# BaratiLab/GAMD

Measured on AMD Instinct MI355X. Metric: atom-steps/sec (force eval + integrate), 10k-atom LJ box, higher is better.
Workload: dtype f32; 1 GPU; C2: 10 000-atom LJ box, rho*=0.5, L=92.29 A, cutoff 3.0 sigma=10.2 A, fp32, 4 conv layers x 128, random-init weights (seed 0), 1 box per GPU; n_atoms=10000, boxes=1, launch=single process

## Files before the change

### gamd_amd/csrc/conv_edge.hip

```cpp
#include "gamd_common.h"
#include "gamd_internal.h"

#include <cstdlib>

namespace {

constexpr int conv_lds_floats(bool l0) { return 2 * GAMD_WFRAG_FLOATS + 3 * 128; }

template <bool F2, typename Post, typename Mid>
__device__ __forceinline__ void gemm128_post(const f32x4* W, int lane, const f32x16 (&X)[4], f32x16 (&acc)[4], Post post, Mid mid) {
#pragma unroll
    for (int tp = 0; tp < 4; ++tp) {
        if (tp == 1) mid();
#pragma unroll
        for (int t = 0; t < 4; ++t) {
#pragma unroll
            for (int q = 0; q < 4; ++q) {
                const f32x4 w = W[((tp * 4 + t) * 4 + q) * 64 + lane];
#pragma unroll
                for (int j = 0; j < 4; ++j) {
                    const float x = X[t][q * 4 + j];
                    acc[tp] = F2 ? mfma32(x, w[j], acc[tp]) : mfma32(w[j], x, acc[tp]);
                }
                if (tp > 0) post(tp - 1, t * 4 + q);
// ... 8 lines not shown
__device__ __forceinline__ void phase_barrier() {
    asm volatile("s_waitcnt vmcnt(%0) lgkmcnt(0)" ::"n"(N) : "memory");
    __builtin_amdgcn_s_barrier();
}

__device__ __forceinline__ void load_e_tile(const float* __restrict__ e_frag, int tile, int lane, f32x16 (&X)[4]) {
    const f32x4* ef = (const f32x4*)e_frag + (size_t)tile * 16 * 64;
#pragma unroll
    for (int t = 0; t < 4; ++t)
#pragma unroll
        for (int q = 0; q < 4; ++q) {
            const f32x4 v = gamd_load_stream(&ef[(t * 4 + q) * 64 + lane]);
#pragma unroll
            for (int j = 0; j < 4; ++j) X[t][q * 4 + j] = v[j];
        }
}

template <bool TIME, bool L0>
__global__ void __launch_bounds__(512, 2) k_conv_edge(ConvEdgeArgs a) {
    if (a.devflags[DEVFLAG_FROZEN]) return;
    extern __shared__ __attribute__((aligned(16))) float lds[];
    float* buf0 = lds + (L0 ? 3 * 128 : 0);
    float* buf1 = buf0 + GAMD_WFRAG_FLOATS;
    float* vb1 = L0 ? lds : buf1 + GAMD_WFRAG_FLOATS;
    float* vb3 = vb1 + 128;
    float* vb4 = vb3 + 128;
    float* vSD0 = vb4;

    const int tid = threadIdx.x, lane = tid & 63, slot = lane & 31, half = lane >> 5;
    const int wave = __builtin_amdgcn_readfirstlane(tid >> 6);
    const unsigned lane16 = (unsigned)lane * 16u;
    int E = a.counters[CNT_E];
    if ((long long)E > a.e_cap) E = (int)a.e_cap;
    const int n_tiles = (E + GAMD_TILE - 1) / GAMD_TILE;
    const int n_units = (n_tiles + 3) / 4;
    int first, end, step;
    gamd_xcd_range(n_units, blockIdx.x, gridDim.x, first, end, step);
    if (first >= end) return;
    const int n_iter = ((end - first + step - 1) / step + 1) / 2;
    const int wsub = wave & 3, whalf = wave >> 2;
    const bool early = whalf == 0;
    auto tile_of = [&](int it) {
        const int u = first + (2 * it + whalf) * step;
        return (it < n_iter && u < end) ? u * 4 + wsub : n_tiles;
    };
    auto stage = [&](const float* gw, float* buf) { gamd_stage_weight_raw_contig<8>(gw, buf, wave, lane16); };

    long long tacc[16];
#pragma unroll
    for (int i = 0; i < 16; ++i) tacc[i] = 0;
    long long tprev = 0;
#define TMARK(i) do { if (TIME) { const long long tn__ = (long long)__builtin_readcyclecounter(); tacc[i] += tn__ - tprev; tprev = tn__; } } while (0)

    if (tid < 128) {
        vb1[tid] = a.b1[tid]; vb3[tid] = a.b3[tid];
        if (L0) vSD0[tid] = a.S[tid] + a.D[tid];
        else vb4[tid] = a.b4[tid];
    }
    stage(a.w1p, buf0);

    f32x16 RA[4], RB[4], RC[4];
    auto init_b4 = [&]() {
#pragma unroll
        for (int tp = 0; tp < 4; ++tp) {
            const float b = vb4[32 * tp + slot];
#pragma unroll
            for (int r = 0; r < 16; ++r) RC[tp][r] = b;
        }
    };

    int tile = tile_of(0);
    bool active = tile < n_tiles;
    int src = 0, dst = 0;
    {
// ... 101 lines not shown
        asm volatile("" ::"v"(mask), "v"(p0), "v"(src_n));
        TMARK(5);
        if (active) {
            const unsigned bl = (unsigned)__ballot(src != a.zero_row) >> (4 * half);
            const unsigned real = (bl & 0xFu) | ((bl >> 4) & 0xF0u) | ((bl >> 8) & 0xF00u) | ((bl >> 12) & 0xF000u);
#pragma unroll
            for (int tp = 0; tp < 4; ++tp) {
                const float b = vb3[32 * tp + slot];
#pragma unroll
                for (int r = 0; r < 16; ++r) RC[tp][r] = ((real >> r) & 1u) ? b : GAMD_L0_PAD;
            }
            TMARK(7);
            const unsigned keep_bits = ~(mask << 1);
            gemm128_post<true>((const f32x4*)bx, lane, RA, RC, [&](int tp, int r) {
                RC[tp][r] = gamd_l0_acc(RC[tp][r], (r > 0 && ((keep_bits >> r) & 1u)) ? RC[tp][r - 1] : 0.f);
            }, [&]() { FENCE(); if (it + 1 < n_iter) stage(a.w1p, by); FENCE(); });
            pend_ends = mask;
            if (nvalid > 0 && !((mask >> (nvalid - 1)) & 1u)) pend_ends |= 1u << (nvalid - 1);
            pend_p = p0;
            TMARK(10);
        } else {
            if (it + 1 < n_iter) stage(a.w1p, by);
        }
        if (!early) phase_barrier<0>();
        TMARK(11);
        if (active_n) load_e_tile(a.e_frag, tile_n, lane, RA);
        TMARK(12);
        if (early) early_barrier(active_n);
        TMARK(13);
        tile = tile_n; active = active_n; src = src_n;
    }
    } else {
    for (int it = 0; it < n_iter; ++it) {
        const int x0 = tile * GAMD_TILE + 16 * half;
        int nvalid = E - x0;
        nvalid = !active ? 0 : (nvalid >= 16 ? 16 : (nvalid <= 0 ? 0 : nvalid));
        const int tile_n = tile_of(it + 1);
// ... 51 lines not shown
            gemm128_post<false>((const f32x4*)buf0, lane, RC, RB,
                                [&](int tp, int g) { RB[tp][g] = gamd_silu_hw(RB[tp][g]); },
                                [&]() { FENCE(); stage(a.w4p, buf1); FENCE(); });
            TMARK(8);
        } else {
            stage(a.w4p, buf1);
        }
        phase_barrier<0>();
        asm volatile("" ::"v"(mask), "v"(p0), "v"(src_n), "v"(dst_n));
        TMARK(9);
        if (active) {
            init_b4();
            const unsigned keep_bits = ~(mask << 1);
            gemm128_post<true>((const f32x4*)buf1, lane, RB, RC, [&](int tp, int r) {
                RC[tp][r] = gamd_msg_acc(RA[r >> 2][(r & 3) * 4 + tp], RC[tp][r], (r > 0 && ((keep_bits >> r) & 1u)) ? RC[tp][r - 1] : 0.f);
            }, [&]() { FENCE(); if (it + 1 < n_iter) stage(a.w1p, buf0); FENCE(); });
            pend_ends = mask;
            if (nvalid > 0 && !((mask >> (nvalid - 1)) & 1u)) pend_ends |= 1u << (nvalid - 1);
            pend_p = p0;
            TMARK(10);
        } else {
            if (it + 1 < n_iter) stage(a.w1p, buf0);
        }
        if (!early) phase_barrier<0>();
        TMARK(11);
        if (active_n) load_e_tile(a.e_frag, tile_n, lane, RA);
        TMARK(12);
        if (early) early_barrier(active_n);
        TMARK(13);
        tile = tile_n; active = active_n; src = src_n; dst = dst_n;
    }
    }
#undef FENCE
    piece_stores();
    if (TIME && a.tdbg && lane == 0) {
#pragma unroll
        for (int i = 0; i < 16; ++i) a.tdbg[((size_t)blockIdx.x * 8 + wave) * 16 + i] = tacc[i];
    }
#undef TMARK
}

template <bool TIME, bool L0>
int launch(const ConvEdgeArgs& a, int n_blocks, hipStream_t st) {
    const size_t lds = sizeof(float) * conv_lds_floats(L0);
    static PerDeviceOnce once;
    if (int e = gamd_allow_dynamic_lds(once, (int)lds, k_conv_edge<TIME, L0>)) return e;
    hipLaunchKernelGGL((k_conv_edge<TIME, L0>), dim3(n_blocks), dim3(512), lds, st, a);
    GAMD_CHECK_LAUNCH();
    return 0;
// ... 20 lines not shown
```

### gamd_amd/csrc/gamd_api.hip

```cpp
#include "gamd_host.h"

#include <algorithm>
#include <cmath>
#include <cstddef>
#include <cstdlib>
#include <cstring>
#include <deque>

static_assert(sizeof(gamd_config) == 96 && offsetof(gamd_config, n_boxes) == 88 && offsetof(gamd_config, edge_capacity) == 40,
              "gamd_config layout is part of the C ABI (gamd_amd/_lib.py mirrors it)");

namespace {

bool small_path(const gamd_handle* h) { return h->use_small; }

int fill_com(gamd_handle* h, int enabled, MdCom* c) {
    c->enabled = enabled ? 1 : 0;
    c->blocks = std::max(1, std::min(16, (h->n_per_box + 1023) / 1024));
    c->partial = nullptr;
    if (!c->enabled) return 0;
    if (h->com_partial.ensure(sizeof(double) * 4 * (size_t)c->blocks * (size_t)h->n_boxes, true)) return fail(-12, "allocation failed");
    c->partial = h->com_partial.as<double>();
    return 0;
}
// ... 424 lines not shown

    for (int l = 0; l < h->L; ++l) {
        ConvEdgeArgs ca{};
        ca.counters = h->cur_counters;
        ca.devflags = h->devflags.as<int>();
        ca.col = h->col.as<int>(); ca.erow = h->erow.as<int>();
        ca.chunk_piece = h->chunk_piece.as<int>(); ca.chunk_mask = h->chunk_mask.as<unsigned>();
        ca.e_frag = (h->update_edge && l > 0) ? h->e_frag2.as<float>() : h->e_frag.as<float>();
        ca.emb_out = (h->update_edge && l + 1 < h->L) ? h->e_emb.as<float>() : nullptr;
        ca.hn = h->hn.as<float>(); ca.S = h->S.as<float>(); ca.D = h->D.as<float>();
        if (l0 && l == 0) { ca.hn = h->l0_hn.as<float>(); ca.S = h->l0_S.as<float>(); ca.D = h->l0_D.as<float>(); }
        const LayerDev& ld = h->layers[l];
        ca.w1p = ld.w1p; ca.w2p = ld.w2p; ca.w3p = ld.w3p; ca.w4p = ld.w4p; ca.w16p = ld.w16p;
        ca.b1 = ld.b1; ca.b3 = ld.b3; ca.b4 = ld.b4;
        const bool hoist = l == 0 && h->l0_hoist;
        if (hoist) { ca.w3p = ld.w3p_l0; ca.b3 = ld.b3_l0; }
        ca.partial = h->partial.as<float>();
        ca.piece_cap = h->piece_cap;
        ca.sticky = h->sticky_dev;
        ca.e_cap = h->e_cap;
        ca.zero_row = h->n;
#ifdef GAMD_CHECKED
        { static const bool inject = getenv("GAMD_CHK_INJECT") != nullptr; if (inject) ca.zero_row = 0; }
#endif
        ca.tdbg = h->tdbg.as<long long>();
        if ((r = tev_begin(l))) return r;
        r = h->DT > 1 ? launch_conv_edge_wide_d(ca, h->EHT, h->HT, h->DT, h->n_cu, st)
            : h->wide_conv ? (h->cfg.edge_dtype == GAMD_EDGE_F16X3 ? launch_conv_edge_f16x3_wide(ca, h->EHT, h->HT, h->n_cu, st)
                            : h->cfg.edge_dtype == GAMD_EDGE_BF16 ? launch_conv_edge_bf16_wide(ca, h->EHT, h->HT, h->n_cu, st)
                            : (half_quantum && ca.w16p && !ca.emb_out) ? launch_conv_edge_wide16(ca, h->EHT, h->HT, h->n_cu, st)
                            : small_tiles > 0 ? launch_conv_edge_small_wide(ca, h->EHT, h->HT, small_tiles, st)
// ... 176 lines not shown
    if (!cfg || !out) return fail(-22, "null argument");
    if (cfg->n_atoms <= 0) return fail(-22, "n_atoms must be positive");
    if (cfg->n_boxes < 0 || cfg->n_boxes > (1 << 20)) return fail(-22, "n_boxes out of range");
    const int n_boxes = cfg->n_boxes > 1 ? cfg->n_boxes : 1;
    if ((long long)cfg->n_atoms * n_boxes >= (1 << 23) - 1)
        return fail(-22, "n_atoms x n_boxes = %lld: at most %d atoms per handle", (long long)cfg->n_atoms * n_boxes, (1 << 23) - 2);
    if (cfg->n_layers <= 0 || cfg->n_layers > 16) return fail(-22, "n_layers out of range");
    if (!(cfg->cutoff > 0.f)) return fail(-22, "cutoff must be positive");
    if (cfg->edge_dtype != GAMD_EDGE_F32 && cfg->edge_dtype != GAMD_EDGE_BF16 && cfg->edge_dtype != GAMD_EDGE_F16X3)
        return fail(-22, "unknown edge_dtype");
    if (!(cfg->neighbor_skin >= 0.f)) return fail(-22, "neighbor_skin must be >= 0");
    if (cfg->self_loop_mode != GAMD_SELF_LOOP_DGL07_NOOP && cfg->self_loop_mode != GAMD_SELF_LOOP_APPEND_ZERO_FEATURE)
        return fail(-22, "unknown self_loop_mode %d", cfg->self_loop_mode);
    if (cfg->self_loop_mode != GAMD_SELF_LOOP_DGL07_NOOP && cfg->edge_dtype != GAMD_EDGE_F32)
        return fail(-22, "self_loop_mode 1 is built for the fp32 edge dtype only");
    if (cfg->kernel_select & ~(GAMD_KSEL_FORCE_GENERIC_WIDTH | GAMD_KSEL_FORCE_HALF_QUANTUM | GAMD_KSEL_NO_LAYER0_HOIST))
        return fail(-22, "unknown kernel_select bits 0x%x", cfg->kernel_select);
    int ndev = 0;
    if (hipGetDeviceCount(&ndev) != hipSuccess || ndev <= 0)
        return fail(-19, "no HIP device available: libgamd_hip has no CPU fallback");
    if (cfg->device < 0 || cfg->device >= ndev) return fail(-22, "device %d out of range (%d visible)", cfg->device, ndev);
    DeviceGuard guard(cfg->device);
    hipDeviceProp_t prop;
    HIP_TRY(hipGetDeviceProperties(&prop, cfg->device));
    const int H_true = cfg->encoding_size ? cfg->encoding_size : 128, Eh_true = cfg->edge_embedding_dim ? cfg->edge_embedding_dim : 128;
    const int D_true = cfg->hidden_dim ? cfg->hidden_dim : 128;
    if (H_true < 1 || H_true > 256 || Eh_true < 1 || Eh_true > 256)
        return fail(-22, "encoding_size and edge_embedding_dim must be in [1, 256] (got %d, %d)", H_true, Eh_true);
    if (D_true < 1 || D_true > 256) return fail(-22, "hidden_dim must be in [1, 256] (got %d)", D_true);
    const int Dp = D_true <= 128 ? 128 : 256;
    if (Dp > 128 && cfg->edge_dtype != GAMD_EDGE_F32)
// ... 145 lines not shown
    h->finalized = false;
    return 0;
}

int32_t gamd_finalize_weights(gamd_handle* h) {
    if (!h) return fail(-22, "null handle");
    DeviceGuard guard(h->dev);
    InitStream init(h->init_stream);
    const int F = h->n_feat, L = h->L;
    const int64_t H = h->H, Eh = h->Eh, HT = h->HT, EHT = h->EHT;
    const int64_t Ht = h->H_true, Et = h->Eh_true, Dt = h->D_true;
    const int64_t Dp = h->Dp, DT = h->DT;
    const bool expand = !h->cfg.no_expand_edge;
    BlobBuilder bb;
    struct Off { size_t w1p, w2p, w3p, w4p, w16p = 0, b1, b3, b4, elng = 0, elnb = 0, lng, lnb, wsp, wdp, wpdp, bS, bP, wpep, wphip, bphi;
                 size_t w3p_l0 = 0, b3_l0 = 0, m0 = 0, c0 = 0; };
    std::vector<Off> lo(L);
    std::deque<HostTensor> padded;
    auto get = [&](const std::string& nm, std::initializer_list<int64_t> shp, std::initializer_list<int64_t> pad) -> const HostTensor* {
        const HostTensor* t = find_w(h, nm, shp);
        if (!t) return nullptr;
        const std::vector<int64_t> ps(pad);
        if (t->shape == ps) return t;
        HostTensor o;
        o.shape = ps;
        const int64_t r = ps.size() == 2 ? t->shape[0] : 1, c = ps.size() == 2 ? t->shape[1] : t->shape[0];
        const int64_t cp = ps.size() == 2 ? ps[1] : ps[0], rp = ps.size() == 2 ? ps[0] : 1;
        o.data.assign((size_t)(rp * cp), 0.f);
        for (int64_t i = 0; i < r; ++i) std::copy(t->data.begin() + i * c, t->data.begin() + (i + 1) * c, o.data.begin() + i * cp);
        padded.push_back(std::move(o));
        return &padded.back();
// ... 55 lines not shown
    h->norm_bn = norm_bn ? 1 : 0;
    h->l0_hoist = h->cfg.kind == GAMD_KIND_LJ && h->cfg.edge_dtype == GAMD_EDGE_F32 && !h->wide_conv && DT == 1 && !update_edge &&
                  !(h->cfg.kernel_select & GAMD_KSEL_NO_LAYER0_HOIST);
    const HostTensor* emb0 = h->l0_hoist ? get("node_emb", {1, Ht}, {1, H}) : nullptr;
    if (h->l0_hoist && !emb0) return -2;
    auto permute_f2 = [](const HostTensor& w, const HostTensor& b, HostTensor& wo, HostTensor& bo) {
        wo = w;
        bo = b;
        for (int q = 0; q < 4; ++q)
            for (int s = 0; s < 32; ++s) {
                std::copy(w.data.begin() + (size_t)(4 * s + q) * 128, w.data.begin() + (size_t)(4 * s + q + 1) * 128,
                          wo.data.begin() + (size_t)(32 * q + s) * 128);
                bo.data[32 * q + s] = b.data[4 * s + q];
            }
    };
    for (int l = 0; l < L; ++l) {
        const std::string p = "graph_conv.conv." + std::to_string(l);
        const HostTensor *ea0w = get(p + ".edge_affine.mlp_layer.0.weight", {128, Et}, {128, Eh}), *ea0b = get(p + ".edge_affine.mlp_layer.0.bias", {128}, {128});
        const HostTensor *ea2w = get(p + ".edge_affine.mlp_layer.2.weight", {Dt, 128}, {Dp, 128}), *ea2b = get(p + ".edge_affine.mlp_layer.2.bias", {Dt}, {Dp});
        const HostTensor *sw = get(p + ".src_affine.weight", {Dt, Ht}, {Dp, H}), *sb = get(p + ".src_affine.bias", {Dt}, {Dp});
        const HostTensor *dw = get(p + ".dst_affine.weight", {Dt, Ht}, {Dp, H}), *db = get(p + ".dst_affine.bias", {Dt}, {Dp});
        const HostTensor *t1w = get(p + ".theta_edge.mlp_layer.1.weight", {Dt, Dt}, {Dp, Dp}), *t1b = get(p + ".theta_edge.mlp_layer.1.bias", {Dt}, {Dp});
        const HostTensor *t3w = get(p + ".theta_edge.mlp_layer.3.weight", {Ht, Dt}, {H, Dp}), *t3b = get(p + ".theta_edge.mlp_layer.3.bias", {Ht}, {H});
        const HostTensor *pdw = get(p + ".phi_dst.weight", {Dt, Ht}, {Dp, H}), *pdb = get(p + ".phi_dst.bias", {Dt}, {Dp});
        const HostTensor *pew = get(p + ".phi_edge.weight", {Dt, Ht}, {Dp, H}), *peb = get(p + ".phi_edge.bias", {Dt}, {Dp});
        const HostTensor *phw = get(p + ".phi.mlp_layer.1.weight", {Ht, Dt}, {H, Dp}), *phb = get(p + ".phi.mlp_layer.1.bias", {Ht}, {H});
        const HostTensor *ng = get("graph_conv.norm_layers." + std::to_string(l) + ".weight", {Ht}, {H});
        const HostTensor *nb = get("graph_conv.norm_layers." + std::to_string(l) + ".bias", {Ht}, {H});
        if (!ea0w || !ea0b || !ea2w || !ea2b || !sw || !sb || !dw || !db || !t1w || !t1b || !t3w || !t3b || !pdw ||
            !pdb || !pew || !peb || !phw || !phb || !ng || !nb)
// ... 50 lines not shown
                std::fill(row.begin(), row.end(), 0.0);
                double cr = 0.0;
                for (int64_t i = 0; i < H; ++i) {
                    const double a = (double)pew->data[(size_t)(r * H + i)] * hn0[i];
                    if (a == 0.0) continue;
                    for (int64_t k = 0; k < Dp; ++k) row[k] += a * t3w->data[(size_t)(i * Dp + k)];
                    cr += a * t3b->data[i];
                }
                for (int64_t k = 0; k < Dp; ++k) m0.data[(size_t)(r * Dp + k)] = (float)row[k];
                c0.data[r] = (float)cr;
            }
            HostTensor w3f, b3f;
            permute_f2(*t1w, *t1b, w3f, b3f);
            o.w3p_l0 = put_blocks(&w3f, 1, 1);
            o.b3_l0 = put_vec(&b3f);
            o.m0 = put_node(&m0, 1, 1);
            o.c0 = put_vec(&c0);
        }
        HostTensor b4_perm;
        HostTensor w4_perm;
        auto permute_w4 = [&]() {
            permute_f2(*t3w, *t3b, w4_perm, b4_perm);
            t3b = &b4_perm;
        };
        if (bf16_edges) {
            permute_w4();
            o.w1p = put_edge_bf16(ea0w); o.w2p = put_edge_bf16(ea2w); o.w3p = put_edge_bf16(t1w); o.w4p = put_edge_bf16(&w4_perm);
        } else if (f16x3_edges) {
            o.w1p = put_edge_f16x3(ea0w); o.w2p = put_edge_f16x3(ea2w); o.w3p = put_edge_f16x3(t1w); o.w4p = put_edge_f16x3(t3w);
        } else if (bf16_wide) {
// ... 19 lines not shown
            o.w2p = put_blocks(ea2w, (int)DT, 1);
            o.w3p = put_blocks(t1w, (int)DT, (int)DT);
            if (DT > 1) {
                o.w4p = put_blocks(t3w, (int)HT, (int)DT);
            } else if (h->wide_conv) {
                o.w4p = put_blocks(t3w, (int)HT, 1);
                o.w16p = bb.add((size_t)(EHT + 2 + HT) * GAMD_WFRAG_FLOATS);
                size_t at = o.w16p;
                for (int kb = 0; kb < (int)EHT; ++kb, at += GAMD_WFRAG_FLOATS) pack16x(ea0w->data.data() + 128 * kb, bb.host.data() + at, 128 * (int)EHT, true);
                pack16x(ea2w->data.data(), bb.host.data() + at, 128, true); at += GAMD_WFRAG_FLOATS;
                pack16x(t1w->data.data(), bb.host.data() + at, 128, true); at += GAMD_WFRAG_FLOATS;
                for (int ob = 0; ob < (int)HT; ++ob, at += GAMD_WFRAG_FLOATS) pack16x(t3w->data.data() + (size_t)128 * ob * 128, bb.host.data() + at, 128, false);
            } else {
                permute_w4();
                o.w4p = put_blocks(&w4_perm, 1, 1);
            }
        }
        o.b1 = put_vec(ea0b); o.b3 = put_vec(t1b); o.b4 = put_vec(t3b);
        o.lng = put_vec(ng); o.lnb = put_vec(nb);
        if (update_edge) {
            const HostTensor *eg = get(p + ".edge_layer_norm.weight", {Et}, {Eh}), *eb = get(p + ".edge_layer_norm.bias", {Et}, {Eh});
            if (!eg || !eb) return -2;
            o.elng = put_vec(eg); o.elnb = put_vec(eb);
        }
        o.wsp = put_node(sw, (int)DT, (int)HT); o.wdp = put_node(dw, (int)DT, (int)HT); o.wpdp = put_node(pdw, (int)DT, (int)HT);
        o.bS = bb.add((size_t)Dp);
        for (int i = 0; i < (int)Dp; ++i) bb.host[o.bS + i] = (sb->data[i] + db->data[i]) + ea2b->data[i];
        o.bP = bb.add((size_t)Dp);
        for (int i = 0; i < (int)Dp; ++i) bb.host[o.bP + i] = pdb->data[i] + peb->data[i];
        o.wpep = put_node(pew, (int)DT, (int)HT); o.wphip = put_node(phw, (int)HT, (int)DT); o.bphi = put_vec(phb);
// ... 48 lines not shown
    h->length_mean = lm->data[0];
    h->length_std = ls->data[0];
    h->rbf = RbfGrid{};
    if (expand) {
        const double c0 = cen->data[0], delta = ((double)cen->data[39] - c0) / 39.0;
        bool uniform = delta > 0.0;
        for (int k = 0; k < 40 && uniform; ++k)
            uniform = std::fabs((double)cen->data[k] - (c0 + k * delta)) <= 2.5e-7 * std::max(1.0, std::fabs(c0 + k * delta));
        if (uniform) {
            const double gexp = -(1.0 / 0.025) * 1.4426950408889634, s = 2.0 * delta;
            h->rbf = RbfGrid{1, (float)c0, (float)delta, (float)(-2.0 * gexp * s), (float)(gexp * s * s),
                             (float)std::exp2(2.0 * gexp * s * s)};
        }
    }

    if (h->wblob.ensure(sizeof(float) * bb.host.size(), false)) return fail(-12, "weight blob allocation failed");
    HIP_TRY(init_upload(h->wblob.p, bb.host.data(), sizeof(float) * bb.host.size()));
    const float* B = h->wblob.as<float>();
    h->layers.assign(L, LayerDev{});
    for (int l = 0; l < L; ++l) {
        const Off& o = lo[l];
        LayerDev& d = h->layers[l];
        d.w1p = B + o.w1p; d.w2p = B + o.w2p; d.w3p = B + o.w3p; d.w4p = B + o.w4p;
        d.w16p = (h->wide_conv && h->cfg.edge_dtype == GAMD_EDGE_F32 && DT == 1) ? B + o.w16p : nullptr;
        d.b1 = B + o.b1; d.b3 = B + o.b3; d.b4 = B + o.b4;
        d.node.ln_g = B + o.lng; d.node.ln_b = B + o.lnb;
        if (update_edge) { d.e_ln_g = B + o.elng; d.e_ln_b = B + o.elnb; }
        d.node.wsp = B + o.wsp; d.node.wdp = B + o.wdp; d.node.wpdp = B + o.wpdp;
        d.node.bS = B + o.bS; d.node.bP = B + o.bP;
        d.node.wpep = B + o.wpep; d.node.wphip = B + o.wphip; d.node.bphi = B + o.bphi;
        d.node.c0 = nullptr;
        if (l == 0 && h->l0_hoist) {
            d.w3p_l0 = B + o.w3p_l0; d.b3_l0 = B + o.b3_l0;
            d.node.wpep = B + o.m0; d.node.c0 = B + o.c0;
        }
    }
    h->enc_w1p = B + o_e1; h->enc_w2p = B + o_e2; h->enc_w3p = B + o_e3;
    h->enc_b1 = B + o_eb1; h->enc_b2 = B + o_eb2; h->enc_b3 = B + o_eb3;
    h->enc_lng = B + o_elg; h->enc_lnb = B + o_elb; h->centers = B + o_cen;
    h->dec_w1p = B + o_d1; h->dec_b1 = B + o_db1; h->dec_w2 = B + o_d2; h->dec_b2 = B + o_db2;
    h->node_emb = h->cfg.kind == GAMD_KIND_LJ ? B + o_emb : nullptr;
    h->nenc_w = h->cfg.kind == GAMD_KIND_LJ ? nullptr : B + o_nw;
    h->nenc_b = h->cfg.kind == GAMD_KIND_LJ ? nullptr : B + o_nb;
    h->finalized = true;
    return 0;
}

int32_t gamd_set_scaler(gamd_handle* h, double mean, double var) {
// ... 441 lines not shown
```

### gamd_amd/csrc/gamd_host.h

```cpp
#pragma once
#include "../../include/gamd_hip.h"
#include "gamd_common.h"
#include "gamd_internal.h"

#include <cstdarg>
#include <cstdio>
#include <map>
#include <string>
#include <vector>

#pragma GCC visibility push(hidden)

inline thread_local char g_err[512] = "";

inline int fail(int code, const char* fmt, ...) {
    va_list ap;
    va_start(ap, fmt);
    vsnprintf(g_err, sizeof(g_err), fmt, ap);
    va_end(ap);
    return code;
}

#define HIP_TRY(expr)                                                                              \
    do {                                                                                           \
// ... 30 lines not shown
        bytes = want;
        if (zero) {
            e = hipMemsetAsync(p, 0, want, tl_init_stream);
            if (e == hipSuccess) e = hipStreamSynchronize(tl_init_stream);
            if (e != hipSuccess) return (int)e;
        }
        return 0;
    }
    void release() { if (p) (void)hipFree(p); p = nullptr; bytes = 0; }
    template <typename T> T* as() const { return reinterpret_cast<T*>(p); }
};

struct LayerDev {
    const float *w1p, *w2p, *w3p, *w4p, *b1, *b3, *b4;
    const float *w16p = nullptr;
    const float *e_ln_g = nullptr, *e_ln_b = nullptr;
    const float *w3p_l0 = nullptr, *b3_l0 = nullptr;
    NodeLayerW node;
};

struct DeviceGuard {
    int prev = -1;
    bool changed = false;
    explicit DeviceGuard(int dev) {
        if (hipGetDevice(&prev) == hipSuccess && prev != dev) changed = hipSetDevice(dev) == hipSuccess;
    }
    ~DeviceGuard() { if (changed) (void)hipSetDevice(prev); }
    DeviceGuard(const DeviceGuard&) = delete;
    DeviceGuard& operator=(const DeviceGuard&) = delete;
};
// ... 118 lines not shown
```

### gamd_amd/csrc/wide16.hip

```cpp
#include "gamd_common.h"
#include "gamd_internal.h"

namespace {

__device__ __forceinline__ f32x4 mfma16x(float a, float b, f32x4 c) { return __builtin_amdgcn_mfma_f32_16x16x4f32(a, b, c, 0, 0, 0); }

__device__ __forceinline__ void wide16_barrier() {
    asm volatile("s_waitcnt vmcnt(0) lgkmcnt(0)" ::: "memory");
    __builtin_amdgcn_s_barrier();
    asm volatile("" ::: "memory");
}

template <bool F2, int D = 3>
__device__ __forceinline__ void gemm16x(const f32x4* W, int lane, const f32x4 (&X)[8], f32x4 (&acc)[8]) {
    __builtin_amdgcn_sched_barrier(0);
    f32x4 w0[D], w1[D];
#pragma unroll
    for (int s = 0; s < D; ++s) {
        w0[s] = W[((2 * (s >> 3)) * 8 + (s & 7)) * 64 + lane];
        w1[s] = W[((2 * (s >> 3) + 1) * 8 + (s & 7)) * 64 + lane];
    }
#pragma unroll
    for (int s = 0; s < 32; ++s) {
        const int o2 = s >> 3, m4 = s & 7;
        const f32x4 a0 = w0[s % D], a1 = w1[s % D];
#pragma unroll
        for (int c = 0; c < 4; ++c) {
            const float x = X[m4][c];
            acc[2 * o2] = F2 ? mfma16x(x, a0[c], acc[2 * o2]) : mfma16x(a0[c], x, acc[2 * o2]);
            acc[2 * o2 + 1] = F2 ? mfma16x(x, a1[c], acc[2 * o2 + 1]) : mfma16x(a1[c], x, acc[2 * o2 + 1]);
        }
        if (s + D < 32) {
            const int n = s + D;
            w0[s % D] = W[((2 * (n >> 3)) * 8 + (n & 7)) * 64 + lane];
            w1[s % D] = W[((2 * (n >> 3) + 1) * 8 + (n & 7)) * 64 + lane];
        }
    }
    __builtin_amdgcn_sched_group_barrier(0x100, 2 * D, 0);
#pragma unroll
    for (int s = 0; s < 32 - D; ++s) {
        __builtin_amdgcn_sched_group_barrier(0x008, 8, 0);
        __builtin_amdgcn_sched_group_barrier(0x100, 2, 0);
    }
    __builtin_amdgcn_sched_group_barrier(0x008, 8 * D, 0);
    __builtin_amdgcn_sched_barrier(0);
}

template <typename Ptr>
__device__ __forceinline__ void load_row16x(Ptr row, int g, f32x4 (&X)[8]) {
    const int base = 4 * (g & 1), j0 = g >> 1;
#pragma unroll
    for (int t = 0; t < 4; ++t)
#pragma unroll
        for (int q = 0; q < 4; ++q) {
            const f32x4 v = *reinterpret_cast<const f32x4*>(&row[32 * t + 8 * q + base]);
            const float lo = j0 ? v[1] : v[0], hi = j0 ? v[3] : v[2];
            X[2 * t + (q >> 1)][2 * (q & 1)] = lo;
            X[2 * t + (q >> 1)][2 * (q & 1) + 1] = hi;
        }
}

template <int EHT, int HT>
__global__ void __launch_bounds__(256, 1) k_conv_edge_wide16(ConvEdgeArgs a) {
    if (a.devflags[DEVFLAG_FROZEN]) return;
    constexpr int NP = EHT + 2 + HT;
    constexpr int H = 128 * HT;
    extern __shared__ __attribute__((aligned(16))) float lds[];
    float* vb1 = lds + 2 * GAMD_WFRAG_FLOATS;
    float* vb3 = vb1 + 128;
    float* vb4 = vb3 + 128;

    const int tid = threadIdx.x, lane = tid & 63, la = lane & 15, g = lane >> 4;
    const int wave = __builtin_amdgcn_readfirstlane(tid >> 6);
    const unsigned lane16 = (unsigned)lane * 16u;
    int E = a.counters[CNT_E];
// ... 192 lines not shown
```

### gamd_amd/engine.py

```python
from __future__ import annotations

import ctypes as C
import os
from typing import Dict, Optional, Sequence, Tuple, Union

import numpy as np
import torch

from . import _lib
from ._lib import GamdReportParams, GamdStructParams, GamdTrajParams, GamdConfig, GamdMdParams, GamdNhcParams, TRAJ_FIELDS, check
from .weights import ModelConfig, infer_config, validate_state_dict

ArrayLike = Union[np.ndarray, torch.Tensor]

KIND = {"lj": 0, "water": 1, "dynbox": 1}
FLAVOUR = {"jaxmd": 0, "torch": 1}
SELF_LOOP = {"dgl07_noop": 0, "append_zero_feature_loops": 1}
KSEL_FORCE_GENERIC_WIDTH = 1
KSEL_NO_LAYER0_HOIST = 4


def _box3(box) -> np.ndarray:
    b = np.asarray(box, dtype=np.float64).reshape(-1)
    if b.size == 1:
        b = np.repeat(b, 3)
    if b.size != 3:
        raise ValueError("box must be a scalar or 3 values")
    return b.astype(np.float32)


def _boxes(box, n_boxes: int) -> np.ndarray:
    b = np.asarray(box, dtype=np.float64)
    if b.ndim == 0 or b.size == 1 or (b.ndim == 1 and b.size == 3):
        return np.tile(_box3(b), (n_boxes, 1))
# ... 663 lines not shown
```

### include/gamd_hip.h

```cpp
#ifndef GAMD_HIP_H
#define GAMD_HIP_H

#include <stdint.h>
#include <stddef.h>

#ifdef __cplusplus
extern "C" {
#endif

typedef struct gamd_handle gamd_handle;

enum { GAMD_EDGE_F32 = 0, GAMD_EDGE_BF16 = 1, GAMD_EDGE_F16X3 = 2 };

enum { GAMD_KIND_LJ = 0, GAMD_KIND_WATER = 1 };
enum { GAMD_NBR_JAXMD = 0, GAMD_NBR_TORCH = 1 };

typedef struct gamd_config {
    int32_t n_atoms;
    int32_t kind;
    int32_t n_layers;
    int32_t use_bond;
    int32_t nbr_flavour;
    int32_t device;
    float cutoff;
    float box[3];
    int64_t edge_capacity;
    int32_t keep_stages;
    int32_t edge_dtype;
    int32_t encoding_size;
    int32_t edge_embedding_dim;
    int32_t hidden_dim;
    int32_t no_expand_edge;
    float neighbor_skin;
    int32_t self_loop_mode;
    int32_t kernel_select;
    int32_t small_tile_limit;
    int32_t n_boxes;
} gamd_config;
enum { GAMD_SELF_LOOP_DGL07_NOOP = 0, GAMD_SELF_LOOP_APPEND_ZERO_FEATURE = 1 };
enum { GAMD_KSEL_FORCE_GENERIC_WIDTH = 1, GAMD_KSEL_FORCE_HALF_QUANTUM = 2, GAMD_KSEL_NO_LAYER0_HOIST = 4 };

const char* gamd_version(void);
const char* gamd_last_error(void);

int32_t gamd_create(const gamd_config* cfg, gamd_handle** out);
int32_t gamd_destroy(gamd_handle* h);

int32_t gamd_load_weight(gamd_handle* h, const char* name, const float* data, const int64_t* shape, int32_t ndim);
int32_t gamd_finalize_weights(gamd_handle* h);

int32_t gamd_set_scaler(gamd_handle* h, double mean, double var);

int32_t gamd_set_bonds(gamd_handle* h, const int32_t* bonds, int64_t n_bonds);

int32_t gamd_forces_async(gamd_handle* h, const float* pos_dev, const uint8_t* species_dev, const float* box,
// ... 130 lines not shown
```

Baseline: 3.375 million atom-steps/s.

## Spread conv-edge tail units across blocks as 16-edge chunks

```diff
diff --git a/gamd_amd/csrc/conv_edge.hip b/gamd_amd/csrc/conv_edge.hip
--- a/gamd_amd/csrc/conv_edge.hip
+++ b/gamd_amd/csrc/conv_edge.hip
@@ -1,4 +1,5 @@
 #include "gamd_common.h"
+#include "gamd_chain16x.h"
 #include "gamd_internal.h"
 
 #include <cstdlib>
@@ -46,6 +47,93 @@
 #pragma unroll
             for (int j = 0; j < 4; ++j) X[t][q * 4 + j] = v[j];
         }
+}
+
+template <bool L0, typename Flush>
+__device__ __forceinline__ void conv_tail16(const ConvEdgeArgs& a, int E, int n_tiles, int chunk0, float* wa, float* wb, const float* vb1,
+                                            const float* vb3, const float* vb4, int wave, int lane, unsigned lane16, Flush flush) {
+    const int la = lane & 15, g = lane >> 4;
+    const int chunk = chunk0 + wave;
+    const bool mine = wave < 4 && chunk < 2 * n_tiles;
+    auto stage = [&](int blk, float* buf) { gamd_stage_weight_raw_contig<8>(a.w16p + (size_t)blk * GAMD_WFRAG_FLOATS, buf, wave, lane16); };
+    int src = a.zero_row, dst = a.zero_row, nvalid = 0, p0 = 0;
+    unsigned mask = 0;
+    f32x4 X[8], T[8], U[8], SQ[8], HN[4][2];
+    if (mine) {
+        const int x = chunk * GAMD_CHUNK + la;
+        if (x < E) {
+            src = GAMD_CHK_RANGE(a.sticky, a.col[x], 0, a.zero_row, GAMD_CHK_CONV_SRC);
+            if (!L0) dst = GAMD_CHK_RANGE(a.sticky, a.erow[x], 0, a.zero_row, GAMD_CHK_CONV_DST);
+        }
+        const int nv = E - chunk * GAMD_CHUNK;
+        nvalid = nv >= 16 ? 16 : (nv <= 0 ? 0 : nv);
+        mask = a.chunk_mask[chunk];
+        p0 = GAMD_CHK_RANGE(a.sticky, a.chunk_piece[chunk], 0, a.piece_cap - 17, GAMD_CHK_PIECE);
+        load_e16x((const f32x4*)a.e_frag + (size_t)(chunk >> 1) * 16 * 64, chunk & 1, la, g, X);
+    }
+    flush();
+    if (mine && !L0) {
+        load_row16x(a.S + (size_t)src * GAMD_H, g, SQ);
+        load_row16x(a.D + (size_t)dst * GAMD_H, g, U);
+        load_hn16x(a.hn, GAMD_H, src, la, g, HN);
+    }
+    stage(1, wb);
+    if (mine) {
+        load_row16x(vb1, g, T);
+        gemm16x<false>((const f32x4*)wa, lane, X, T);
+#pragma unroll
+        for (int o = 0; o < 8; ++o)
+#pragma unroll
+            for (int r = 0; r < 4; ++r) T[o][r] = gamd_silu_hw(T[o][r]);
+    }
+    wide16_barrier();
+    stage(2, wa);
+    if (mine) {
+        if (L0) load_row16x(vb4, g, U);
+        gemm16x<false>((const f32x4*)wb, lane, T, U);
+#pragma unroll
+        for (int o = 0; o < 8; ++o)
+#pragma unroll
+            for (int r = 0; r < 4; ++r) U[o][r] = gamd_silu_hw(L0 ? U[o][r] : U[o][r] + SQ[o][r]);
+    }
+    wide16_barrier();
+    if constexpr (L0) {
+        if (mine) {
+            const unsigned real = (unsigned)__ballot(src != a.zero_row);
+#pragma unroll
+            for (int ob = 0; ob < 8; ++ob) {
+                const float b = vb3[32 * (ob & 3) + 16 * (ob >> 2) + la];
+#pragma unroll
+                for (int r = 0; r < 4; ++r) X[ob][r] = ((real >> (4 * g + r)) & 1u) ? b : GAMD_L0_PAD;
+            }
+            gemm16x<true>((const f32x4*)wa, lane, U, X);
+            segsum16x(X, mask, lane, g, [&](int, int, int, float pre, float prev) { return gamd_l0_acc(pre, prev); });
+            store_pieces16x(a.partial, GAMD_H, X, mask, nvalid, p0, la, g);
+        }
+    } else {
+        stage(3, wb);
+        if (mine) {
+            load_row16x(vb3, g, T);
+            gemm16x<false>((const f32x4*)wa, lane, U, T);
+#pragma unroll
+            for (int o = 0; o < 8; ++o)
+#pragma unroll
+                for (int r = 0; r < 4; ++r) T[o][r] = gamd_silu_hw(T[o][r]);
+        }
+        wide16_barrier();
+        if (mine) {
+#pragma unroll
+            for (int ob = 0; ob < 8; ++ob) {
+                const float b = vb4[32 * (ob & 3) + 16 * (ob >> 2) + la];
+                X[ob] = f32x4{b, b, b, b};
+            }
+            gemm16x<true>((const f32x4*)wb, lane, T, X);
+            segsum16x(X, mask, lane, g, [&](int ob, int r, int e, float e_emb, float prev) {
+                return gamd_msg_acc((e < nvalid) ? HN[r][ob >> 2][ob & 3] : 0.f, e_emb, prev);
+            });
+            store_pieces16x(a.partial, GAMD_H, X, mask, nvalid, p0, la, g);
+        }
+    }
 }
 
 template <bool TIME, bool L0>
@@ -68,8 +156,17 @@
     const int n_units = (n_tiles + 3) / 4;
     int first, end, step;
     gamd_xcd_range(n_units, blockIdx.x, gridDim.x, first, end, step);
-    if (first >= end) return;
-    const int n_iter = ((end - first + step - 1) / step + 1) / 2;
+    int tail_chunk = -1;
+    if (a.w16p && gridDim.x >= 8 && gridDim.x % 8 == 0) {
+        const int w = blockIdx.x / 8, lo = first - w, cnt = end - lo;
+        const int c_min = cnt / step, rem = cnt - c_min * step;
+        if (rem > 0 && 8 * rem <= 4 * step) {
+            end = lo + c_min * step;
+            if (w < 2 * rem) tail_chunk = 8 * end + 4 * w;
+        }
+    }
+    if (first >= end && tail_chunk < 0) return;
+    const int n_iter = first < end ? ((end - first + step - 1) / step + 1) / 2 : 0;
     const int wsub = wave & 3, whalf = wave >> 2;
     const bool early = whalf == 0;
     auto tile_of = [&](int it) {
@@ -77,6 +174,7 @@
         return (it < n_iter && u < end) ? u * 4 + wsub : n_tiles;
     };
     auto stage = [&](const float* gw, float* buf) { gamd_stage_weight_raw_contig<8>(gw, buf, wave, lane16); };
+    auto stage_w1 = [&](int it, float* buf) { if (it + 1 < n_iter) stage(a.w1p, buf); else if (tail_chunk >= 0) stage(a.w16p, buf); };
 
     long long tacc[16];
 #pragma unroll
@@ -89,7 +187,7 @@
         if (L0) vSD0[tid] = a.S[tid] + a.D[tid];
         else vb4[tid] = a.b4[tid];
     }
-    stage(a.w1p, buf0);
+    stage(n_iter > 0 ? a.w1p : a.w16p, buf0);
 
     f32x16 RA[4], RB[4], RC[4];
     auto init_b4 = [&]() {
@@ -221,13 +319,13 @@
             const unsigned keep_bits = ~(mask << 1);
             gemm128_post<true>((const f32x4*)bx, lane, RA, RC, [&](int tp, int r) {
                 RC[tp][r] = gamd_l0_acc(RC[tp][r], (r > 0 && ((keep_bits >> r) & 1u)) ? RC[tp][r - 1] : 0.f);
-            }, [&]() { FENCE(); if (it + 1 < n_iter) stage(a.w1p, by); FENCE(); });
+            }, [&]() { FENCE(); stage_w1(it, by); FENCE(); });
             pend_ends = mask;
             if (nvalid > 0 && !((mask >> (nvalid - 1)) & 1u)) pend_ends |= 1u << (nvalid - 1);
             pend_p = p0;
             TMARK(10);
         } else {
-            if (it + 1 < n_iter) stage(a.w1p, by);
+            stage_w1(it, by);
         }
         if (!early) phase_barrier<0>();
         TMARK(11);
@@ -309,13 +407,13 @@
             const unsigned keep_bits = ~(mask << 1);
             gemm128_post<true>((const f32x4*)buf1, lane, RB, RC, [&](int tp, int r) {
                 RC[tp][r] = gamd_msg_acc(RA[r >> 2][(r & 3) * 4 + tp], RC[tp][r], (r > 0 && ((keep_bits >> r) & 1u)) ? RC[tp][r - 1] : 0.f);
-            }, [&]() { FENCE(); if (it + 1 < n_iter) stage(a.w1p, buf0); FENCE(); });
+            }, [&]() { FENCE(); stage_w1(it, buf0); FENCE(); });
             pend_ends = mask;
             if (nvalid > 0 && !((mask >> (nvalid - 1)) & 1u)) pend_ends |= 1u << (nvalid - 1);
             pend_p = p0;
             TMARK(10);
         } else {
-            if (it + 1 < n_iter) stage(a.w1p, buf0);
+            stage_w1(it, buf0);
         }
         if (!early) phase_barrier<0>();
         TMARK(11);
@@ -327,7 +425,12 @@
     }
     }
 #undef FENCE
-    piece_stores();
+    if (tail_chunk >= 0) {
+        float* const wa = (L0 && (n_iter & 1)) ? buf1 : buf0;
+        conv_tail16<L0>(a, E, n_tiles, tail_chunk, wa, wa == buf0 ? buf1 : buf0, vb1, vb3, vb4, wave, lane, lane16, piece_stores);
+    } else {
+        piece_stores();
+    }
     if (TIME && a.tdbg && lane == 0) {
 #pragma unroll
         for (int i = 0; i < 16; ++i) a.tdbg[((size_t)blockIdx.x * 8 + wave) * 16 + i] = tacc[i];
diff --git a/gamd_amd/csrc/gamd_api.hip b/gamd_amd/csrc/gamd_api.hip
--- a/gamd_amd/csrc/gamd_api.hip
+++ b/gamd_amd/csrc/gamd_api.hip
@@ -462,7 +462,8 @@
         ca.w1p = ld.w1p; ca.w2p = ld.w2p; ca.w3p = ld.w3p; ca.w4p = ld.w4p; ca.w16p = ld.w16p;
         ca.b1 = ld.b1; ca.b3 = ld.b3; ca.b4 = ld.b4;
         const bool hoist = l == 0 && h->l0_hoist;
-        if (hoist) { ca.w3p = ld.w3p_l0; ca.b3 = ld.b3_l0; }
+        if (hoist) { ca.w3p = ld.w3p_l0; ca.b3 = ld.b3_l0; ca.w16p = ld.w16p_l0; }
+        if (!h->wide_conv && (h->cfg.kernel_select & GAMD_KSEL_NO_CONV_TAIL16)) ca.w16p = nullptr;
         ca.partial = h->partial.as<float>();
         ca.piece_cap = h->piece_cap;
         ca.sticky = h->sticky_dev;
@@ -669,7 +670,7 @@
         return fail(-22, "unknown self_loop_mode %d", cfg->self_loop_mode);
     if (cfg->self_loop_mode != GAMD_SELF_LOOP_DGL07_NOOP && cfg->edge_dtype != GAMD_EDGE_F32)
         return fail(-22, "self_loop_mode 1 is built for the fp32 edge dtype only");
-    if (cfg->kernel_select & ~(GAMD_KSEL_FORCE_GENERIC_WIDTH | GAMD_KSEL_FORCE_HALF_QUANTUM | GAMD_KSEL_NO_LAYER0_HOIST))
+    if (cfg->kernel_select & ~(GAMD_KSEL_FORCE_GENERIC_WIDTH | GAMD_KSEL_FORCE_HALF_QUANTUM | GAMD_KSEL_NO_LAYER0_HOIST | GAMD_KSEL_NO_CONV_TAIL16))
         return fail(-22, "unknown kernel_select bits 0x%x", cfg->kernel_select);
     int ndev = 0;
     if (hipGetDeviceCount(&ndev) != hipSuccess || ndev <= 0)
@@ -845,7 +846,7 @@
     const bool expand = !h->cfg.no_expand_edge;
     BlobBuilder bb;
     struct Off { size_t w1p, w2p, w3p, w4p, w16p = 0, b1, b3, b4, elng = 0, elnb = 0, lng, lnb, wsp, wdp, wpdp, bS, bP, wpep, wphip, bphi;
-                 size_t w3p_l0 = 0, b3_l0 = 0, m0 = 0, c0 = 0; };
+                 size_t w3p_l0 = 0, b3_l0 = 0, w16p_l0 = 0, m0 = 0, c0 = 0; };
     std::vector<Off> lo(L);
     std::deque<HostTensor> padded;
     auto get = [&](const std::string& nm, std::initializer_list<int64_t> shp, std::initializer_list<int64_t> pad) -> const HostTensor* {
@@ -931,6 +932,8 @@
                 bo.data[32 * q + s] = b.data[4 * s + q];
             }
     };
+    struct TailImages { int layer; bool l0; const HostTensor *w1, *w2, *w3, *w4; };
+    std::vector<TailImages> tail_images;
     for (int l = 0; l < L; ++l) {
         const std::string p = "graph_conv.conv." + std::to_string(l);
         const HostTensor *ea0w = get(p + ".edge_affine.mlp_layer.0.weight", {128, Et}, {128, Eh}), *ea0b = get(p + ".edge_affine.mlp_layer.0.bias", {128}, {128});
@@ -1011,6 +1014,7 @@
             permute_f2(*t1w, *t1b, w3f, b3f);
             o.w3p_l0 = put_blocks(&w3f, 1, 1);
             o.b3_l0 = put_vec(&b3f);
+            tail_images.push_back(TailImages{l, true, ea0w, ea2w, t1w, nullptr});
             o.m0 = put_node(&m0, 1, 1);
             o.c0 = put_vec(&c0);
         }
@@ -1060,6 +1064,7 @@
             } else {
                 permute_w4();
                 o.w4p = put_blocks(&w4_perm, 1, 1);
+                tail_images.push_back(TailImages{l, false, ea0w, ea2w, t1w, t3w});
             }
         }
         o.b1 = put_vec(ea0b); o.b3 = put_vec(t1b); o.b4 = put_vec(t3b);
@@ -1138,6 +1143,14 @@
         }
     }
 
+    for (const TailImages& t : tail_images) {
+        const size_t at = bb.add((size_t)(t.l0 ? 3 : 4) * GAMD_WFRAG_FLOATS);
+        (t.l0 ? lo[t.layer].w16p_l0 : lo[t.layer].w16p) = at;
+        pack16x(t.w1->data.data(), bb.host.data() + at, 128, true);
+        pack16x(t.w2->data.data(), bb.host.data() + at + GAMD_WFRAG_FLOATS, 128, true);
+        pack16x(t.w3->data.data(), bb.host.data() + at + 2 * GAMD_WFRAG_FLOATS, 128, !t.l0);
+        if (!t.l0) pack16x(t.w4->data.data(), bb.host.data() + at + 3 * GAMD_WFRAG_FLOATS, 128, false);
+    }
     if (h->wblob.ensure(sizeof(float) * bb.host.size(), false)) return fail(-12, "weight blob allocation failed");
     HIP_TRY(init_upload(h->wblob.p, bb.host.data(), sizeof(float) * bb.host.size()));
     const float* B = h->wblob.as<float>();
@@ -1146,7 +1159,7 @@
         const Off& o = lo[l];
         LayerDev& d = h->layers[l];
         d.w1p = B + o.w1p; d.w2p = B + o.w2p; d.w3p = B + o.w3p; d.w4p = B + o.w4p;
-        d.w16p = (h->wide_conv && h->cfg.edge_dtype == GAMD_EDGE_F32 && DT == 1) ? B + o.w16p : nullptr;
+        d.w16p = (h->cfg.edge_dtype == GAMD_EDGE_F32 && DT == 1) ? B + o.w16p : nullptr;
         d.b1 = B + o.b1; d.b3 = B + o.b3; d.b4 = B + o.b4;
         d.node.ln_g = B + o.lng; d.node.ln_b = B + o.lnb;
         if (update_edge) { d.e_ln_g = B + o.elng; d.e_ln_b = B + o.elnb; }
@@ -1155,7 +1168,7 @@
         d.node.wpep = B + o.wpep; d.node.wphip = B + o.wphip; d.node.bphi = B + o.bphi;
         d.node.c0 = nullptr;
         if (l == 0 && h->l0_hoist) {
-            d.w3p_l0 = B + o.w3p_l0; d.b3_l0 = B + o.b3_l0;
+            d.w3p_l0 = B + o.w3p_l0; d.b3_l0 = B + o.b3_l0; d.w16p_l0 = B + o.w16p_l0;
             d.node.wpep = B + o.m0; d.node.c0 = B + o.c0;
         }
     }
diff --git a/gamd_amd/csrc/gamd_chain16x.h b/gamd_amd/csrc/gamd_chain16x.h
--- /dev/null
+++ b/gamd_amd/csrc/gamd_chain16x.h
@@ -0,0 +1,125 @@
+#pragma once
+#include "gamd_common.h"
+
+__device__ __forceinline__ f32x4 mfma16x(float a, float b, f32x4 c) { return __builtin_amdgcn_mfma_f32_16x16x4f32(a, b, c, 0, 0, 0); }
+
+__device__ __forceinline__ void wide16_barrier() {
+    asm volatile("s_waitcnt vmcnt(0) lgkmcnt(0)" ::: "memory");
+    __builtin_amdgcn_s_barrier();
+    asm volatile("" ::: "memory");
+}
+
+template <bool F2, int D = 3>
+__device__ __forceinline__ void gemm16x(const f32x4* W, int lane, const f32x4 (&X)[8], f32x4 (&acc)[8]) {
+    __builtin_amdgcn_sched_barrier(0);
+    f32x4 w0[D], w1[D];
+#pragma unroll
+    for (int s = 0; s < D; ++s) {
+        w0[s] = W[((2 * (s >> 3)) * 8 + (s & 7)) * 64 + lane];
+        w1[s] = W[((2 * (s >> 3) + 1) * 8 + (s & 7)) * 64 + lane];
+    }
+#pragma unroll
+    for (int s = 0; s < 32; ++s) {
+        const int o2 = s >> 3, m4 = s & 7;
+        const f32x4 a0 = w0[s % D], a1 = w1[s % D];
+#pragma unroll
+        for (int c = 0; c < 4; ++c) {
+            const float x = X[m4][c];
+            acc[2 * o2] = F2 ? mfma16x(x, a0[c], acc[2 * o2]) : mfma16x(a0[c], x, acc[2 * o2]);
+            acc[2 * o2 + 1] = F2 ? mfma16x(x, a1[c], acc[2 * o2 + 1]) : mfma16x(a1[c], x, acc[2 * o2 + 1]);
+        }
+        if (s + D < 32) {
+            const int n = s + D;
+            w0[s % D] = W[((2 * (n >> 3)) * 8 + (n & 7)) * 64 + lane];
+            w1[s % D] = W[((2 * (n >> 3) + 1) * 8 + (n & 7)) * 64 + lane];
+        }
+    }
+    __builtin_amdgcn_sched_group_barrier(0x100, 2 * D, 0);
+#pragma unroll
+    for (int s = 0; s < 32 - D; ++s) {
+        __builtin_amdgcn_sched_group_barrier(0x008, 8, 0);
+        __builtin_amdgcn_sched_group_barrier(0x100, 2, 0);
+    }
+    __builtin_amdgcn_sched_group_barrier(0x008, 8 * D, 0);
+    __builtin_amdgcn_sched_barrier(0);
+}
+
+template <typename Ptr>
+__device__ __forceinline__ void load_row16x(Ptr row, int g, f32x4 (&X)[8]) {
+    const int base = 4 * (g & 1), j0 = g >> 1;
+#pragma unroll
+    for (int t = 0; t < 4; ++t)
+#pragma unroll
+        for (int q = 0; q < 4; ++q) {
+            const f32x4 v = *reinterpret_cast<const f32x4*>(&row[32 * t + 8 * q + base]);
+            const float lo = j0 ? v[1] : v[0], hi = j0 ? v[3] : v[2];
+            X[2 * t + (q >> 1)][2 * (q & 1)] = lo;
+            X[2 * t + (q >> 1)][2 * (q & 1) + 1] = hi;
+        }
+}
+
+__device__ __forceinline__ void load_e16x(const f32x4* ef, int hc, int la, int g, f32x4 (&X)[8]) {
+    ef += 8 * (la >> 2) + 4 * hc + (la & 3) + 32 * (g & 1);
+    const int j0 = g >> 1;
+#pragma unroll
+    for (int t = 0; t < 4; ++t)
+#pragma unroll
+        for (int q = 0; q < 4; ++q) {
+            const f32x4 v = ef[(t * 4 + q) * 64];
+            X[2 * t + (q >> 1)][2 * (q & 1)] = j0 ? v[1] : v[0];
+            X[2 * t + (q >> 1)][2 * (q & 1) + 1] = j0 ? v[3] : v[2];
+        }
+}
+
+__device__ __forceinline__ void load_hn16x(const float* hn128, int H, int src, int la, int g, f32x4 (&HN)[4][2]) {
+#pragma unroll
+    for (int r = 0; r < 4; ++r) {
+        const int sr = __shfl(src, 4 * g + r, 64);
+        const float* hrow = hn128 + (size_t)sr * H + 4 * la;
+        HN[r][0] = *reinterpret_cast<const f32x4*>(hrow);
+        HN[r][1] = *reinterpret_cast<const f32x4*>(hrow + 64);
+    }
+}
+
+template <typename Step>
+__device__ __forceinline__ void segsum16x(f32x4 (&X)[8], unsigned mask, int lane, int g, Step step) {
+    const unsigned keep_bits = ~(mask << 1);
+#pragma unroll
+    for (int gg = 0; gg < 4; ++gg) {
+        float cin[8];
+#pragma unroll
+        for (int ob = 0; ob < 8; ++ob) {
+            const float last = X[ob][3];
+            cin[ob] = gg == 0 ? 0.f : __shfl(last, lane - 16, 64);
+        }
+        if (g == gg) {
+#pragma unroll
+            for (int ob = 0; ob < 8; ++ob) {
+                float run = cin[ob];
+                float o4[4];
+#pragma unroll
+                for (int r = 0; r < 4; ++r) {
+                    const int e = 4 * gg + r;
+                    run = step(ob, r, e, X[ob][r], (e > 0 && ((keep_bits >> e) & 1u)) ? run : 0.f);
+                    o4[r] = run;
+                }
+                X[ob] = f32x4{o4[0], o4[1], o4[2], o4[3]};
+            }
+        }
+    }
+}
+
+__device__ __forceinline__ void store_pieces16x(float* prow0, int H, const f32x4 (&X)[8], unsigned mask, int nvalid, int p0, int la, int g) {
+    unsigned ends = mask;
+    if (nvalid > 0 && !((mask >> (nvalid - 1)) & 1u)) ends |= 1u << (nvalid - 1);
+#pragma unroll
+    for (int r = 0; r < 4; ++r) {
+        const int e = 4 * g + r;
+        if ((ends >> e) & 1u) {
+            const int p = p0 + __popc(ends & ((1u << e) - 1u));
+            float* prow = prow0 + (size_t)p * H + 4 * la;
+            *reinterpret_cast<f32x4*>(prow) = f32x4{X[0][r], X[1][r], X[2][r], X[3][r]};
+            *reinterpret_cast<f32x4*>(prow + 64) = f32x4{X[4][r], X[5][r], X[6][r], X[7][r]};
+        }
+    }
+}
diff --git a/gamd_amd/csrc/gamd_host.h b/gamd_amd/csrc/gamd_host.h
--- a/gamd_amd/csrc/gamd_host.h
+++ b/gamd_amd/csrc/gamd_host.h
@@ -68,6 +68,7 @@
 struct LayerDev {
     const float *w1p, *w2p, *w3p, *w4p, *b1, *b3, *b4;
     const float *w16p = nullptr;
+    const float *w16p_l0 = nullptr;
     const float *e_ln_g = nullptr, *e_ln_b = nullptr;
     const float *w3p_l0 = nullptr, *b3_l0 = nullptr;
     NodeLayerW node;
diff --git a/gamd_amd/csrc/wide16.hip b/gamd_amd/csrc/wide16.hip
--- a/gamd_amd/csrc/wide16.hip
+++ b/gamd_amd/csrc/wide16.hip
@@ -1,64 +1,8 @@
 #include "gamd_common.h"
+#include "gamd_chain16x.h"
 #include "gamd_internal.h"
 
 namespace {
-
-__device__ __forceinline__ f32x4 mfma16x(float a, float b, f32x4 c) { return __builtin_amdgcn_mfma_f32_16x16x4f32(a, b, c, 0, 0, 0); }
-
-__device__ __forceinline__ void wide16_barrier() {
-    asm volatile("s_waitcnt vmcnt(0) lgkmcnt(0)" ::: "memory");
-    __builtin_amdgcn_s_barrier();
-    asm volatile("" ::: "memory");
-}
-
-template <bool F2, int D = 3>
-__device__ __forceinline__ void gemm16x(const f32x4* W, int lane, const f32x4 (&X)[8], f32x4 (&acc)[8]) {
-    __builtin_amdgcn_sched_barrier(0);
-    f32x4 w0[D], w1[D];
-#pragma unroll
-    for (int s = 0; s < D; ++s) {
-        w0[s] = W[((2 * (s >> 3)) * 8 + (s & 7)) * 64 + lane];
-        w1[s] = W[((2 * (s >> 3) + 1) * 8 + (s & 7)) * 64 + lane];
-    }
-#pragma unroll
-    for (int s = 0; s < 32; ++s) {
-        const int o2 = s >> 3, m4 = s & 7;
-        const f32x4 a0 = w0[s % D], a1 = w1[s % D];
-#pragma unroll
-        for (int c = 0; c < 4; ++c) {
-            const float x = X[m4][c];
-            acc[2 * o2] = F2 ? mfma16x(x, a0[c], acc[2 * o2]) : mfma16x(a0[c], x, acc[2 * o2]);
-            acc[2 * o2 + 1] = F2 ? mfma16x(x, a1[c], acc[2 * o2 + 1]) : mfma16x(a1[c], x, acc[2 * o2 + 1]);
-        }
-        if (s + D < 32) {
-            const int n = s + D;
-            w0[s % D] = W[((2 * (n >> 3)) * 8 + (n & 7)) * 64 + lane];
-            w1[s % D] = W[((2 * (n >> 3) + 1) * 8 + (n & 7)) * 64 + lane];
-        }
-    }
-    __builtin_amdgcn_sched_group_barrier(0x100, 2 * D, 0);
-#pragma unroll
-    for (int s = 0; s < 32 - D; ++s) {
-        __builtin_amdgcn_sched_group_barrier(0x008, 8, 0);
-        __builtin_amdgcn_sched_group_barrier(0x100, 2, 0);
-    }
-    __builtin_amdgcn_sched_group_barrier(0x008, 8 * D, 0);
-    __builtin_amdgcn_sched_barrier(0);
-}
-
-template <typename Ptr>
-__device__ __forceinline__ void load_row16x(Ptr row, int g, f32x4 (&X)[8]) {
-    const int base = 4 * (g & 1), j0 = g >> 1;
-#pragma unroll
-    for (int t = 0; t < 4; ++t)
-#pragma unroll
-        for (int q = 0; q < 4; ++q) {
-            const f32x4 v = *reinterpret_cast<const f32x4*>(&row[32 * t + 8 * q + base]);
-            const float lo = j0 ? v[1] : v[0], hi = j0 ? v[3] : v[2];
-            X[2 * t + (q >> 1)][2 * (q & 1)] = lo;
-            X[2 * t + (q >> 1)][2 * (q & 1) + 1] = hi;
-        }
-}
 
 template <int EHT, int HT>
 __global__ void __launch_bounds__(256, 1) k_conv_edge_wide16(ConvEdgeArgs a) {
diff --git a/gamd_amd/engine.py b/gamd_amd/engine.py
--- a/gamd_amd/engine.py
+++ b/gamd_amd/engine.py
@@ -18,6 +18,7 @@
 SELF_LOOP = {"dgl07_noop": 0, "append_zero_feature_loops": 1}
 KSEL_FORCE_GENERIC_WIDTH = 1
 KSEL_NO_LAYER0_HOIST = 4
+KSEL_NO_CONV_TAIL16 = 8
 
 
 def _box3(box) -> np.ndarray:
diff --git a/include/gamd_hip.h b/include/gamd_hip.h
--- a/include/gamd_hip.h
+++ b/include/gamd_hip.h
@@ -38,7 +38,8 @@
     int32_t n_boxes;
 } gamd_config;
 enum { GAMD_SELF_LOOP_DGL07_NOOP = 0, GAMD_SELF_LOOP_APPEND_ZERO_FEATURE = 1 };
-enum { GAMD_KSEL_FORCE_GENERIC_WIDTH = 1, GAMD_KSEL_FORCE_HALF_QUANTUM = 2, GAMD_KSEL_NO_LAYER0_HOIST = 4 };
+enum { GAMD_KSEL_FORCE_GENERIC_WIDTH = 1, GAMD_KSEL_FORCE_HALF_QUANTUM = 2, GAMD_KSEL_NO_LAYER0_HOIST = 4,
+       GAMD_KSEL_NO_CONV_TAIL16 = 8 };
 
 const char* gamd_version(void);
 const char* gamd_last_error(void);
```

Result: no change. 3.378 million atom-steps/s (median of 3 runs) (+0.1%).
